# KdaiP/StableTTS

Hardware: AMD Instinct MI355X
Metric: mel-frames/sec (whole node), 31M DiT, n_timesteps=10+CFG (higher is better)
Workload: dtype f16

## Files before the change

stabletts_amd/csrc/attention.hip:

```cpp
#include "common.h"
#include "launch.h"

#if (defined(ST_ABL_NOEXP) || defined(ST_ABL_NOSUM)) && !defined(ST_DEVTOOLS)
#error "ST_ABL_* (ablation builds: results are garbage) need -DST_DEVTOOLS"
#endif
#ifdef ST_ABL_NOEXP
constexpr bool kAblNoExp = true;
#else
constexpr bool kAblNoExp = false;
#endif
#ifdef ST_ABL_NOSUM
constexpr bool kAblNoSum = true;
#else
constexpr bool kAblNoSum = false;
#endif
#ifndef ST_ATTN_WAVES
#define ST_ATTN_WAVES 8
#endif

namespace st {

template <class P, bool TRAIN, bool SPLIT = false, bool VLO = false>
__global__ __launch_bounds__(64 * ST_ATTN_WAVES, ST_ATTN_WAVES >= 16 || SPLIT ? 2 : 4) void attention_kernel(const AttnArgs a) {
    static_assert(!(TRAIN && SPLIT), "split-precision scores: inference kernel only");
    static_assert(!VLO || (TRAIN && !SPLIT), "hi + lo v: training kernel only");
    constexpr bool X3 = SPLIT || VLO;
    constexpr int NW = ST_ATTN_WAVES, QB = 32 * NW, QTILE = QB;
    using vec8 = typename P::vec8;
    constexpr int TILE_BYTES = 64 * 128;
    constexpr int NBUF = 3;
    constexpr int NT = X3 ? 3 : 2;
    constexpr int SMEM = NT * NBUF * TILE_BYTES > NW * 32 * 144 ? NT * NBUF * TILE_BYTES : NW * 32 * 144;
    __shared__ __attribute__((aligned(16))) unsigned char smem[SMEM];
    __shared__ float wave_lse[NW];
    unsigned char* Ks = smem;
    unsigned char* Vs = smem + NBUF * TILE_BYTES;
    unsigned char* KLs = smem + 2 * NBUF * TILE_BYTES;
    unsigned char* VLs = KLs;

    const int T = a.T, Tp = a.Tp, H = a.H;
    const int qtiles = (T + QB - 1) / QB;
    const int j = blockIdx.x >> 3;
    const int qt = j % qtiles, nh = (j / qtiles) * 8 + (blockIdx.x & 7);
    if (nh >= a.n_items * H) return;
    const int n = nh / H, h = nh % H;
    const int mb = n % a.mask_mod;
    if (a.t_lim && qt * QTILE >= a.t_lim[mb]) return;
    const int kvend = a.kv_end[mb];
    const int nfull = a.n_full[mb];
    const float* kbias = a.kbias + (size_t)mb * Tp;

    const int tid = threadIdx.x, lane = tid & 63;
    const int wave = __builtin_amdgcn_readfirstlane(tid >> 6);
    const int l31 = lane & 31, hi = lane >> 5;
    const int query = qt * QB + wave * 32 + l31;

    const unsigned char* qbase = (const unsigned char*)a.q + ((size_t)nh * T) * 128;
    const unsigned char* kbase = (const unsigned char*)a.k + ((size_t)nh * T) * 128;
    const unsigned char* vbase = (const unsigned char*)a.vt + ((size_t)nh * 64) * Tp * 2;
    const unsigned char* qlbase = SPLIT ? (const unsigned char*)a.q_lo + ((size_t)nh * T) * 128 : nullptr;
    const unsigned char* klbase = SPLIT ? (const unsigned char*)a.k_lo + ((size_t)nh * T) * 128 : nullptr;
    const unsigned char* vlbase = VLO ? (const unsigned char*)a.vt_lo + ((size_t)nh * 64) * Tp * 2 : nullptr;
    if constexpr (TRAIN) {
        if (qt * QB >= kvend) {
            if (query < T) {
                unsigned char* orow = (unsigned char*)a.out + (((size_t)n * T + query) * (H * 64) + h * 64) * 2 + hi * 64;
#pragma unroll
                for (int i = 0; i < 4; ++i) *(uint4*)(orow + 16 * i) = make_uint4(0, 0, 0, 0);
                if (hi == 0) a.lse[(size_t)nh * T + query] = 0.f;
            }
            return;
        }
    }

    vec8 qf[4];
#pragma unroll
    for (int ks = 0; ks < 4; ++ks) {
        uint4 v = make_uint4(0, 0, 0, 0);
        if (query < T) v = *(const uint4*)(qbase + (size_t)query * 128 + ks * 32 + hi * 16);
        qf[ks] = as_vec8<P>(v);
    }
    vec8 qlf[SPLIT ? 4 : 1];
    if constexpr (SPLIT) {
#pragma unroll
        for (int ks = 0; ks < 4; ++ks) {
            uint4 v = make_uint4(0, 0, 0, 0);
            if (query < T) v = *(const uint4*)(qlbase + (size_t)query * 128 + ks * 32 + hi * 16);
            qlf[ks] = as_vec8<P>(v);
        }
    }

    const int ntiles = (kvend + 63) >> 6;
    auto sgpr_ptr = [](const unsigned char* p) {
        const uintptr_t v = (uintptr_t)p;
        return (const unsigned char*)(((uintptr_t)(unsigned)__builtin_amdgcn_readfirstlane((int)(v >> 32)) << 32) |
                                      (unsigned)__builtin_amdgcn_readfirstlane((int)(unsigned)v));
    };
    auto issueKV = [&](int kt, int buf) {
        auto k_piece = [&](int piece) {
            int ln = lane;
            if constexpr (TRAIN) asm volatile("" : "+v"(ln));
            const int row = piece * 8 + (ln >> 3);
            const int seg = (ln & 7) ^ ((row >> 1) & 7);
            const int key = min(kt * 64 + row, T - 1);
            glds16s(sgpr_ptr(kbase), (unsigned)(key * 128 + seg * 16), Ks + buf * TILE_BYTES + piece * 1024);
            if constexpr (SPLIT) glds16s(sgpr_ptr(klbase), (unsigned)(key * 128 + seg * 16), KLs + buf * TILE_BYTES + piece * 1024);
        };
        auto v_piece = [&](int piece) {
            const int row = piece * 8 + (lane >> 3);
            const int seg = (lane & 7) ^ ((row >> 1) & 7);
            glds16s(sgpr_ptr(vbase + (size_t)kt * 128), (unsigned)((row * Tp + seg * 8) * 2), Vs + buf * TILE_BYTES + piece * 1024);
            if constexpr (VLO) glds16s(sgpr_ptr(vlbase + (size_t)kt * 128), (unsigned)((row * Tp + seg * 8) * 2), VLs + buf * TILE_BYTES + piece * 1024);
        };
        if constexpr (NW <= 8) {
#pragma unroll
            for (int k = 0; k < 8 / NW; ++k) { k_piece(wave * (8 / NW) + k); v_piece(wave * (8 / NW) + k); }
        } else {
            if (wave < 8) k_piece(wave); else v_piece(wave - 8);
        }
    };

    int row_off[2], swz[2];
#pragma unroll
    for (int b = 0; b < 2; ++b) {
        const int row = b * 32 + l31;
        row_off[b] = row * 128; swz[b] = (row >> 1) & 7;
    }

    f32x16_t o[2];
#pragma unroll
    for (int d = 0; d < 2; ++d)
#pragma unroll
        for (int r = 0; r < 16; ++r) o[d][r] = 0.f;
    constexpr float kBig = 8192.0f, kLazyTrain = 8.0f, kFloor = -20000.0f;
    unsigned drop_rh = 0;
    if constexpr (TRAIN) { if (a.drop.thresh16) drop_rh = a.drop.rowh[(size_t)nh * T + (query < T ? query : T - 1)]; }
    float m_ref = 0.f, l_run = 0.f;
    vec8 qaug, kaug;
#pragma unroll
    for (int i = 0; i < 8; ++i) { qaug[i] = to16<P>(0.f); kaug[i] = to16<P>(0.f); }
    if (hi == 0) kaug[0] = to16<P>(1.0f);

    if (ntiles > 0) issueKV(0, 0);
    if (ntiles > 1) { issueKV(1, 1); if constexpr (NW <= 8) { if constexpr (NW == 8) { if constexpr (X3) ST_DMA_WAIT(3); else ST_DMA_WAIT(2); } else { if constexpr (X3) ST_DMA_WAIT(6); else ST_DMA_WAIT(4); } } else ST_DMA_WAIT(1); }
    else ST_DMA_WAIT(0);
    __syncthreads();

    const int ntiles_run = ntiles;
    bool dead = false;
    if constexpr (!TRAIN) dead = a.t_lim && qt * QB + wave * 32 >= a.t_lim[mb];
    int buf = 0;
    for (int kt = 0; kt < ntiles_run; ++kt) {
        if (kt + 2 < ntiles_run) issueKV(kt + 2, buf >= 1 ? buf - 1 : NBUF - 1);
        if (!dead) {

        f32x16_t s[2];
        const bool partial = (kt + 1) * 64 > nfull;
        auto scores = [&]() __attribute__((always_inline)) {
#pragma unroll
            for (int kb = 0; kb < 2; ++kb) {
#pragma unroll
                for (int r = 0; r < 16; ++r) s[kb][r] = 0.f;
                s[kb] = P::mfma(kaug, qaug, s[kb]);
                const unsigned char* kp = Ks + buf * TILE_BYTES + row_off[kb];
#pragma unroll
                for (int ks = 0; ks < 4; ++ks) {
                    const vec8 kfrag = as_vec8<P>(*(const uint4*)(kp + (((ks * 2 + hi) ^ swz[kb]) << 4)));
                    s[kb] = P::mfma(kfrag, qf[ks], s[kb]);
                    if constexpr (SPLIT) {
                        s[kb] = P::mfma(kfrag, qlf[ks], s[kb]);
                        const unsigned char* klp = KLs + buf * TILE_BYTES + row_off[kb];
                        s[kb] = P::mfma(as_vec8<P>(*(const uint4*)(klp + (((ks * 2 + hi) ^ swz[kb]) << 4))), qf[ks], s[kb]);
                    }
                }
                __builtin_amdgcn_sched_barrier(0);
            }
            if (partial) {
#pragma unroll
                for (int kb = 0; kb < 2; ++kb)
#pragma unroll
                    for (int g4 = 0; g4 < 4; ++g4) {
                        const float4 bz = *(const float4*)(kbias + kt * 64 + kb * 32 + 8 * g4 + 4 * hi);
                        s[kb][4 * g4 + 0] += bz.x; s[kb][4 * g4 + 1] += bz.y;
                        s[kb][4 * g4 + 2] += bz.z; s[kb][4 * g4 + 3] += bz.w;
                    }
            }
        };
        vec8 pf[4];
        float psum[2];
        scores();
        if constexpr (TRAIN) {
            float mx = s[0][0];
#pragma unroll
            for (int kb = 0; kb < 2; ++kb)
#pragma unroll
                for (int r = 0; r < 16; ++r) mx = fmaxf(mx, s[kb][r]);
            mx = xor32_max(mx);
            if (kt == 0 || __any(mx > kLazyTrain)) {
                const bool need = kt == 0 || mx > kLazyTrain;
                const float m_new = need ? (float)to16<P>(fmaxf(m_ref + mx, kFloor)) : m_ref;
                const float alpha = kt == 0 ? 1.0f : __builtin_amdgcn_exp2f(m_ref - m_new);
                l_run *= alpha;
#pragma unroll
                for (int d = 0; d < 2; ++d)
#pragma unroll
                    for (int r = 0; r < 16; ++r) o[d][r] *= alpha;
                m_ref = m_new;
                if (hi == 0) qaug[0] = to16<P>(-m_ref);
                scores();
            }
            psum[0] = 0.f; psum[1] = 0.f;
#pragma unroll
            for (int kb = 0; kb < 2; ++kb)
#pragma unroll
                for (int g4 = 0; g4 < 4; ++g4) {
                    if (g4 == 2) __builtin_amdgcn_sched_barrier(0);
                    uint2 ch = make_uint2(0u, 0u);
                    if (a.drop.thresh16) ch = *(const uint2*)(a.drop.colh + ((kt * 64 + kb * 32 + 8 * g4 + 4 * hi) >> 1));
#pragma unroll
                    for (int h2 = 0; h2 < 2; ++h2) {
                        const int r = 4 * g4 + 2 * h2;
                        float p0 = __builtin_amdgcn_exp2f(s[kb][r]), p1 = __builtin_amdgcn_exp2f(s[kb][r + 1]);
                        psum[0] = add_f32_asm_safe(psum[0], p0);
                        psum[1] = add_f32_asm_safe(psum[1], p1);
                        if (a.drop.thresh16) {
                            const float2 f = drop_factors2(a.drop, drop_pair(drop_rh, h2 ? ch.y : ch.x));
                            p0 *= f.x; p1 *= f.y;
                        }
                        pf[kb * 2 + (r >> 3)][r & 7] = to16<P>(p0);
                        pf[kb * 2 + (r >> 3)][(r & 7) + 1] = to16<P>(p1);
                    }
                }
        } else {
            auto raise = [&](bool first) __attribute__((always_inline)) {
                float mx = s[0][0];
#pragma unroll
                for (int kb = 0; kb < 2; ++kb)
#pragma unroll
                    for (int r = 0; r < 16; ++r) mx = fmaxf(mx, s[kb][r]);
                mx = xor32_max(mx);
                const bool need = first || mx > 0.0f;
                const float m_new = need ? (float)to16<P>(fmaxf(m_ref + mx, kFloor)) : m_ref;
                const float alpha = first ? 1.0f : __builtin_amdgcn_exp2f(m_ref - m_new);
                l_run *= alpha;
#pragma unroll
                for (int d = 0; d < 2; ++d)
#pragma unroll
                    for (int r = 0; r < 16; ++r) o[d][r] *= alpha;
                m_ref = m_new;
                if (hi == 0) qaug[0] = to16<P>(-m_ref);
                scores();
            };
            auto numerators = [&]() __attribute__((always_inline)) {
                psum[0] = 0.f; psum[1] = 0.f;
#pragma unroll
                for (int kb = 0; kb < 2; ++kb)
#pragma unroll
                    for (int r = 0; r < 16; r += 2) {
                        float p0, p1;
                        if constexpr (kAblNoExp) { p0 = s[kb][r] * 0.001f; p1 = s[kb][r + 1] * 0.001f; }
                        else { p0 = __builtin_amdgcn_exp2f(s[kb][r]); p1 = __builtin_amdgcn_exp2f(s[kb][r + 1]); }
                        if constexpr (!kAblNoSum) {
                            psum[0] = add_f32_scalar(psum[0], p0);
                            psum[1] = add_f32_scalar(psum[1], p1);
                        }
                        pf[kb * 2 + (r >> 3)][r & 7] = to16<P>(p0);
                        pf[kb * 2 + (r >> 3)][(r & 7) + 1] = to16<P>(p1);
                    }
            };
            if (kt == 0) raise(true);
            numerators();
            if (kt != 0 && __any(!(psum[0] + psum[1] <= kBig))) {
                scores();
                raise(false);
                numerators();
            }
        }
        l_run += psum[0] + psum[1];

        __builtin_amdgcn_sched_barrier(0);
#pragma unroll
        for (int d = 0; d < 2; ++d) {
            const unsigned char* vp = Vs + buf * TILE_BYTES + row_off[d];
#pragma unroll
            for (int g = 0; g < 4; ++g)
                o[d] = P::mfma(as_vec8<P>(*(const uint4*)(vp + (((g * 2 + hi) ^ swz[d]) << 4))), pf[g], o[d]);
            if constexpr (VLO) {
                const unsigned char* vlp = VLs + buf * TILE_BYTES + row_off[d];
#pragma unroll
                for (int g = 0; g < 4; ++g)
                    o[d] = P::mfma(as_vec8<P>(*(const uint4*)(vlp + (((g * 2 + hi) ^ swz[d]) << 4))), pf[g], o[d]);
            }
        }
        }
        if (kt + 2 < ntiles_run) { if constexpr (NW <= 8) { if constexpr (NW == 8) { if constexpr (X3) ST_DMA_WAIT(3); else ST_DMA_WAIT(2); } else { if constexpr (X3) ST_DMA_WAIT(6); else ST_DMA_WAIT(4); } } else ST_DMA_WAIT(1); }
        else ST_DMA_WAIT(0);
        __syncthreads();
        buf = buf == NBUF - 1 ? 0 : buf + 1;
    }
    const float m_run = m_ref;
    const float l_tot = xor32_sum(l_run);
    const float inv = l_tot > 0.f ? 1.0f / l_tot : 0.f;
    if constexpr (!TRAIN) {
        if (a.lse_max) {
            float v = -3.0e38f;
            if (!dead && query < T && query < kvend && l_tot > 0.f) v = m_run + log2f(l_tot);
#pragma unroll
            for (int off = 16; off > 0; off >>= 1) v = fmaxf(v, __shfl_xor(v, off));
            if (lane == 0) wave_lse[wave] = v;
            __syncthreads();
            if (tid == 0) {
                float b = wave_lse[0];
#pragma unroll
                for (int w = 1; w < NW; ++w) b = fmaxf(b, wave_lse[w]);
                int bits = __float_as_int(b);
                bits = bits >= 0 ? bits : bits ^ 0x7fffffff;
                atomicMax((int*)a.lse_max + ((blockIdx.x % kLseCells) << 4), bits);
            }
        }
    }
    if (dead) return;
    if constexpr (TRAIN) {
        int lane_q = lane;
        asm volatile("" : "+v"(lane_q));
        const int query_e = qt * QB + wave * 32 + (lane_q & 31);
        if ((lane_q >> 5) == 0 && query_e < T) a.lse[(size_t)nh * T + query_e] = l_tot > 0.f ? m_run + log2f(l_tot) : 0.f;
    }
    unsigned char* mine = smem + wave * (32 * 144);
#pragma unroll
    for (int d = 0; d < 2; ++d)
#pragma unroll
        for (int q4 = 0; q4 < 4; ++q4)
            *(uint2*)(mine + l31 * 144 + (d * 32 + 8 * q4 + 4 * hi) * 2) =
                pack4<P>(o[d][4 * q4 + 0] * inv, o[d][4 * q4 + 1] * inv, o[d][4 * q4 + 2] * inv, o[d][4 * q4 + 3] * inv);
    const int rsub = lane >> 3, seg = lane & 7;
    unsigned char* obase = (unsigned char*)a.out + (((size_t)n * T + qt * QB + wave * 32) * (H * 64) + h * 64) * 2 + seg * 16;
#pragma unroll
    for (int i = 0; i < 4; ++i) {
        const int row = i * 8 + rsub;
        const uint4 v = *(const uint4*)(mine + row * 144 + seg * 16);
        if (qt * QB + wave * 32 + row < T) *(uint4*)(obase + (size_t)row * (H * 64) * 2) = v;
    }
}

constexpr int kAttnSmallLds = 8 * 2 * 64 * 128;
template <class P>
__global__ __launch_bounds__(512, 1) void attention_small_kernel(const AttnArgs a) {
    constexpr int NW = 8, TILE_BYTES = 64 * 128, WAVE_LDS = 2 * TILE_BYTES, OP = 33, QTILE = 32;
    using vec8 = typename P::vec8;
    extern __shared__ __attribute__((aligned(16))) unsigned char smem[];

    const int T = a.T, Tp = a.Tp, H = a.H;
    const int qgroups = (T + 31) / 32;
    const int total = a.n_items * H * qgroups;
    const int per_xcd = gridDim.x >> 3;
    const int lin = (blockIdx.x & 7) * per_xcd + (blockIdx.x >> 3);
    if (lin >= total) return;
    const int qt = lin % qgroups;
    const int nh = lin / qgroups;
    const int n = nh / H, h = nh % H;
    const int mb = n % a.mask_mod;
    if (a.t_lim && qt * QTILE >= a.t_lim[mb]) return;
    const int kvend = a.kv_end[mb];
    const int nfull = a.n_full[mb];
    const float* kbias = a.kbias + (size_t)mb * Tp;

    const int tid = threadIdx.x, lane = tid & 63;
    const int wave = __builtin_amdgcn_readfirstlane(tid >> 6);
    const int l31 = lane & 31, hi = lane >> 5;
    const int query = qt * 32 + l31;

    const unsigned char* qbase = (const unsigned char*)a.q + ((size_t)nh * T) * 128;
    const unsigned char* kbase = (const unsigned char*)a.k + ((size_t)nh * T) * 128;
    const unsigned char* vbase = (const unsigned char*)a.vt + ((size_t)nh * 64) * Tp * 2;
    const unsigned char* zeros = (const unsigned char*)a.zeros;
    unsigned char* Ks = smem + wave * WAVE_LDS;
    unsigned char* Vs = Ks + TILE_BYTES;
// ... 103 lines not shown
#pragma unroll
    for (int w = 0; w < NW; ++w) { mw[w] = ((const float*)(smem + w * WAVE_LDS))[64 * OP + q]; M = fmaxf(M, mw[w]); }
    float L = 0.f, acc[4] = {0.f, 0.f, 0.f, 0.f};
#pragma unroll
    for (int w = 0; w < NW; ++w) {
        const float* pw = (const float*)(smem + w * WAVE_LDS);
        const float sc = __builtin_amdgcn_exp2f(mw[w] - M);
        L += pw[64 * OP + 32 + q] * sc;
#pragma unroll
        for (int i = 0; i < 4; ++i) acc[i] += pw[(d0 + i) * OP + q] * sc;
    }
    const float inv = L > 0.f ? 1.0f / L : 0.f;
    if (qt * 32 + q < T)
        *(uint2*)((unsigned char*)a.out + (((size_t)n * T + qt * 32 + q) * (H * 64) + h * 64 + d0) * 2) =
            pack4<P>(acc[0] * inv, acc[1] * inv, acc[2] * inv, acc[3] * inv);
    if (a.lse_max) {
        __shared__ float wave_lse[NW];
        float v = -3.0e38f;
        if (qt * 32 + q < T && qt * 32 + q < kvend && L > 0.f) v = M + log2f(L);
#pragma unroll
        for (int off = 32; off > 0; off >>= 1) v = fmaxf(v, __shfl_xor(v, off));
        if (lane == 0) wave_lse[wave] = v;
        __syncthreads();
        if (tid == 0) {
            float b = wave_lse[0];
#pragma unroll
            for (int w = 1; w < NW; ++w) b = fmaxf(b, wave_lse[w]);
            int bits = __float_as_int(b);
            bits = bits >= 0 ? bits : bits ^ 0x7fffffff;
            atomicMax((int*)a.lse_max + ((blockIdx.x % kLseCells) << 4), bits);
        }
    }
}

template <class P>
static hipError_t launch_attention_small(const AttnArgs& a, hipStream_t s) {
    static bool attr_done_dev[64] = {};
    int dev_ = 0;
    if (hipGetDevice(&dev_) != hipSuccess || dev_ < 0 || dev_ >= 64) return hipErrorInvalidDevice;
    if (!attr_done_dev[dev_]) {
        hipError_t e = hipFuncSetAttribute((const void*)attention_small_kernel<P>, hipFuncAttributeMaxDynamicSharedMemorySize, kAttnSmallLds);
        if (e != hipSuccess) return e;
        attr_done_dev[dev_] = true;
    }
    const int total = a.n_items * a.H * ((a.T + 31) / 32);
    const int grid = ((total + 7) / 8) * 8;
    hipLaunchKernelGGL((attention_small_kernel<P>), dim3(grid), dim3(512), kAttnSmallLds, s, a);
    return hipGetLastError();
}

hipError_t launch_attention(int dtype, const AttnArgs& a, hipStream_t s) {
    if (!a.zeros || !a.kbias) return hipErrorInvalidValue;
    const int qtiles = (a.T + 32 * ST_ATTN_WAVES - 1) / (32 * ST_ATTN_WAVES);
    const int total = a.n_items * a.H * qtiles;
    if (!a.lse && !a.q_lo && a.small_max_blocks > 0 && total <= a.small_max_blocks)
        return dtype == DT_BF16 ? launch_attention_small<OpBF16>(a, s) : launch_attention_small<OpF16>(a, s);
    const int grid = 8 * ((a.n_items * a.H + 7) / 8) * qtiles;
    if (a.lse) {
        if (a.vt_lo) {
            if (dtype == DT_BF16) hipLaunchKernelGGL((attention_kernel<OpBF16, true, false, true>), dim3(grid), dim3(64 * ST_ATTN_WAVES), 0, s, a);
            else                  hipLaunchKernelGGL((attention_kernel<OpF16, true, false, true>), dim3(grid), dim3(64 * ST_ATTN_WAVES), 0, s, a);
            return hipGetLastError();
        }
        if (dtype == DT_BF16) hipLaunchKernelGGL((attention_kernel<OpBF16, true>), dim3(grid), dim3(64 * ST_ATTN_WAVES), 0, s, a);
        else                  hipLaunchKernelGGL((attention_kernel<OpF16, true>), dim3(grid), dim3(64 * ST_ATTN_WAVES), 0, s, a);
        return hipGetLastError();
    }
    if (a.q_lo || a.k_lo) {
        if (!a.q_lo || !a.k_lo) return hipErrorInvalidValue;
        static bool attr_done_dev[64][2] = {};
        int dev_ = 0;
        if (hipGetDevice(&dev_) != hipSuccess || dev_ < 0 || dev_ >= 64) return hipErrorInvalidDevice;
        const int di = dtype == DT_BF16 ? 0 : 1;
        const void* fn = di == 0 ? (const void*)attention_kernel<OpBF16, false, true> : (const void*)attention_kernel<OpF16, false, true>;
        if (!attr_done_dev[dev_][di]) {
            hipError_t e = hipFuncSetAttribute(fn, hipFuncAttributeMaxDynamicSharedMemorySize, 0);
            (void)e;
            attr_done_dev[dev_][di] = true;
        }
        if (di == 0) hipLaunchKernelGGL((attention_kernel<OpBF16, false, true>), dim3(grid), dim3(64 * ST_ATTN_WAVES), 0, s, a);
        else         hipLaunchKernelGGL((attention_kernel<OpF16, false, true>), dim3(grid), dim3(64 * ST_ATTN_WAVES), 0, s, a);
        return hipGetLastError();
    }
    if (dtype == DT_BF16) hipLaunchKernelGGL((attention_kernel<OpBF16, false>), dim3(grid), dim3(64 * ST_ATTN_WAVES), 0, s, a);
    else                  hipLaunchKernelGGL((attention_kernel<OpF16, false>), dim3(grid), dim3(64 * ST_ATTN_WAVES), 0, s, a);
    return hipGetLastError();
}

}
```

stabletts_amd/csrc/engine.cpp:

```cpp
#include "engine_dit.h"
#include "train_launch.h"
#include "mas_launch.h"
#include "align_train_launch.h"

#include <algorithm>
#include <cmath>
#include <cstdio>
#include <cstring>
#include <map>
#include <string>
#include <vector>

using namespace st;
using namespace sthost;

namespace sthost {
std::string g_create_error;

const char* kProfNames[PC_COUNT] = {
    "prep", "prenet_conv", "in_proj", "film_ln1", "qkv_rope", "attention", "out_proj", "ln2",
    "ffn_conv1", "ffn_conv2", "lsc_conv", "final_proj", "ode_update", "train_forward", "train_backward"};

int dev_alloc(st_engine* e, void** p, size_t bytes) {
    HIPCHK(e, hipMalloc(p, bytes ? bytes : 16));
// ... 341 lines not shown
    for (int i = 0; i < dit->L; ++i) {
        const std::string pre = "blocks." + std::to_string(i) + ".time_fusion.film.";
        HIPCHK(e, launch_linear(p.tau, p.n_t, C, P(e, pre + "weight"), P(e, pre + "bias"), 2 * C,
                                p.film + (size_t)i * p.n_t * 2 * C, 0, 0, s));
    }
    return ST_OK;
}

int run_estimator(st_engine* e, const Plan& p, const float* mask, int ev, hipStream_t s) {
    DitState* dit = dit_of(e);
    const int C = dit->C, F = dit->F, L = dit->L, N = p.N, T = p.T;
    const int64_t rowsC = (int64_t)N * T * C;
    const bool cap = e->capture;
    const bool dec = e->kind == KIND_DECODER;
    const bool film = dec;
    const bool skips = dec;
    const bool dec_fast_paths = dec;
    const bool split_qk = dec_fast_paths && dit->attn_split;
    const bool ragged = dec_fast_paths && e->tile.ragged_skip && !cap;
    const int ln1_by_ffn = skips ? L / 2 : L;
    auto ada_of = [&](int i) { return p.ada + (size_t)i * N * 6 * C; };
    auto fuse_ln1 = [&](ConvGemmArgs& a, int i) {
        a.ln_film = nullptr; a.ln_film_stride = 0; a.ln_film_mod = 1;
        if (film) {
            const float* fb = p.film + (size_t)i * p.n_t * 2 * C;
            if (ev >= 0) a.ln_film = fb + (size_t)ev * 2 * C;
            else         { a.ln_film = fb; a.ln_film_stride = 2 * C; a.ln_film_mod = p.B; }
        }
        a.ln_ada = ada_of(i); a.ln_ada_stride = 6 * C; a.ln_shift_off = 0; a.ln_scale_off = C;
        a.ln_mask_out = 0; a.ln_h16 = p.h16; a.mask = mask;
    };
    if (film) {
        ConvGemmArgs a = base_args(e, p, dit->inx, N);
        a.a0 = p.x16; a.c0 = dit->Mp; a.a0_mod = p.B; a.a1 = p.x16lo; a.c1 = dit->Mp; a.a1_mod = p.B; a.c2 = dit->Mp;
        a.bias = nullptr;
        a.add32 = p.cpart; a.add_clamp = p.B;
        a.out32 = p.X; a.out16 = p.skip16[0];
        fuse_ln1(a, 0);
        ProfScope ps(e, s, PC_INPROJ, conv_flops(p, dit->inx, N));
        HIPCHK(e, gemm(e, 1, EPI_F32, a, s));
    } else {
        FilmLnArgs a; memset(&a, 0, sizeof(a));
        a.X = p.X; a.h16 = p.h16; a.film = nullptr; a.film_mod = 1;
        a.ada = ada_of(0); a.ada_stride = 6 * C; a.shift_off = 0; a.scale_off = C;
        a.mask = mask; a.mask_mod = p.B; a.mask_out = 0; a.T = T; a.rows = N * T;
        ProfScope ps(e, s, PC_FILM_LN1, 0);
        HIPCHK(e, launch_film_ln(e->dt, a, s));
    }
    if (film && cap) capture(e, "h0", p.skip16[0], rowsC, true, s);
    for (int i = 0; i < L; ++i) {
        const std::string bn = "b" + std::to_string(i) + ".";
        const float* ada_i = ada_of(i);
        if (skips && i >= L / 2) {
            const int j = i - L / 2;
            ConvGemmArgs a = base_args(e, p, dit->lsc[j], N);
            a.a0 = p.cur16; a.c0 = C; a.a1 = p.skip16[L - 1 - i]; a.c1 = C;
            a.out32 = p.X;
            fuse_ln1(a, i);
            ProfScope ps(e, s, PC_LSC, conv_flops(p, dit->lsc[j], N));
            if (!(dit->skip_mask >> PC_LSC & 1)) HIPCHK(e, gemm(e, 3, EPI_F32, a, s));
        }
        if (cap) { capture(e, bn + "x1", p.X, rowsC, false, s); capture(e, bn + "h1", p.h16, rowsC, true, s); }
        {
            ConvGemmArgs a = base_args(e, p, dit->qkv[i], N);
            a.a0 = p.h16; a.c0 = C;
            a.q = p.q16; a.k = p.k16; a.vt = p.vt16; a.rope_cos = dit->rope_cos; a.rope_sin = dit->rope_sin;
            if (split_qk) { a.q_lo = p.q16lo; a.k_lo = p.k16lo; }
            a.Tp = p.Tp; a.n_heads = dit->H;
            if ((int)dit->qkv_frag.size() == L) a.w_frag = dit->qkv_frag[i];
            a.qscale = 1.4426950408889634f / sqrtf((float)(C / dit->H));
            ProfScope ps(e, s, PC_QKV, conv_flops(p, dit->qkv[i], N));
            if (!(dit->skip_mask >> PC_QKV & 1)) HIPCHK(e, gemm(e, 1, EPI_QKV, a, s));
        }
        if (cap) {
            capture(e, bn + "q", p.q16, rowsC, true, s); capture(e, bn + "k", p.k16, rowsC, true, s);
            capture(e, bn + "vt", p.vt16, (int64_t)N * C * p.Tp, true, s);
        }
        {
            AttnArgs a; memset(&a, 0, sizeof(a));
            a.q = p.q16; a.k = p.k16; a.vt = p.vt16; a.out = p.ao16; a.kbias = p.kbias; a.mask_mod = p.B; a.zeros = e->zeros;
            a.kv_end = p.kv_end; a.n_full = p.n_full; a.T = T; a.Tp = p.Tp; a.H = dit->H; a.n_items = N;
            a.small_max_blocks = dit->conc == 1 ? dit->attn_small_blocks : 0;
            if (split_qk) { a.q_lo = p.q16lo; a.k_lo = p.k16lo; }
            if (dec_fast_paths) a.lse_max = dit->lse_cells;
            if (ragged) a.t_lim = p.t_lim;
            ProfScope ps(e, s, PC_ATTN, 4.0 * (double)N * dit->H * (double)T * T * (C / dit->H));
            if (!(dit->skip_mask >> PC_ATTN & 1)) HIPCHK(e, launch_attention(e->dt, a, s));
        }
        if (cap) capture(e, bn + "attn", p.ao16, rowsC, true, s);
        const bool fused = dec_fast_paths && dit->fused_ffn && !cap && (int)dit->ffn_stream.size() == L && dit->ffn_stream[i] &&
                           (int64_t)dit->conc * N * ((T + kFfnFusedFrames - 1) / kFfnFusedFrames) >= e->tile.big_min_blocks;
        void* h2buf = fused ? p.h2_16 : p.h16;
        {
            ConvGemmArgs a = base_args(e, p, dit->oproj[i], N);
            a.a0 = p.ao16; a.c0 = C; a.mask = mask; a.gate = ada_i + 2 * C; a.gate_stride = 6 * C; a.out32 = p.X;
            a.ln_h16 = h2buf; a.ln_film = nullptr; a.ln_film_mod = 1;
            a.ln_ada = ada_i; a.ln_ada_stride = 6 * C; a.ln_shift_off = 3 * C; a.ln_scale_off = 4 * C; a.ln_mask_out = 1;
            if (dec_fast_paths && (int)dit->oproj_frag.size() == L && !cap) a.w_frag = dit->oproj_frag[i];
            ProfScope ps(e, s, PC_OPROJ, conv_flops(p, dit->oproj[i], N));
            if (!(dit->skip_mask >> PC_OPROJ & 1)) HIPCHK(e, gemm(e, 1, EPI_RESGATE, a, s));
        }
        if (cap) { capture(e, bn + "x2", p.X, rowsC, false, s); capture(e, bn + "h2", p.h16, rowsC, true, s); }
        if (!fused) {
            ConvGemmArgs a = base_args(e, p, dit->ffn1[i], N);
            a.a0 = p.h16; a.c0 = C; a.mask = mask; a.flags = GF_SILU | GF_MASK; a.out16 = p.u16;
            ProfScope ps(e, s, PC_FFN1, conv_flops(p, dit->ffn1[i], N));
            HIPCHK(e, gemm(e, 3, EPI_ACT16, a, s));
        }
        if (cap) capture(e, bn + "u", p.u16, (int64_t)N * T * F, true, s);
        void* copy16 = (skips && i + 1 < L / 2) ? p.skip16[i + 1] : p.cur16;
        {
            ConvGemmArgs a = base_args(e, p, dit->ffn2[i], N);
            a.a0 = p.u16; a.c0 = F; a.mask = mask; a.gate = ada_i + 5 * C; a.gate_stride = 6 * C; a.out32 = p.X;
            if (fused) { a.a0 = h2buf; a.c0 = C; a.w = dit->ffn_stream[i]; a.bias1 = dit->ffn1[i].bias; a.cmid = F; a.flags = GF_SILU | GF_MASK; }
            a.out16 = copy16;
            if (i + 1 == L) a.out16_lo = p.cur16lo;
            if (i + 1 < ln1_by_ffn) fuse_ln1(a, i + 1);
            else if (dec_fast_paths && !cap) a.out32_readonly = 1;
            ProfScope ps(e, s, PC_FFN2, conv_flops(p, dit->ffn2[i], N) + (fused ? conv_flops(p, dit->ffn1[i], N) : 0.0));
            if (dit->skip_mask >> PC_FFN2 & 1) {}
            else if (fused && dit->fused_ffn == 3) HIPCHK(e, launch_ffn_wino_f16(a, s));
            else if (fused) HIPCHK(e, e->dt == DT_BF16 ? launch_ffn_fused_bf16(a, s) : launch_ffn_fused_f16(a, s));
            else HIPCHK(e, gemm(e, 3, EPI_RESGATE, a, s));
        }
        if (cap) {
            if (film && i + 1 < ln1_by_ffn) capture(e, bn + "x3", copy16, rowsC, true, s);
            else capture(e, bn + "x3", p.X, rowsC, false, s);
        }
    }
    {
        ConvGemmArgs a = base_args(e, p, dit->fin, N);
        a.a0 = p.cur16; a.c0 = C; a.a1 = p.cur16lo; a.c1 = C; a.c2 = C; a.mask = mask; a.flags = GF_MASK; a.out32 = p.v32;
        ProfScope ps(e, s, PC_FINAL, conv_flops(p, dit->fin, N));
        HIPCHK(e, gemm(e, 1, EPI_F32, a, s));
    }
    if (cap) capture(e, "v", p.v32, (int64_t)N * T * dit->Mp, false, s);
    return ST_OK;
}

int check_handle(st_engine* e, Kind kind) {
    if (!e) return ST_ERR_INVALID;
    if (e->kind != kind)
        return e->fail(ST_ERR_STATE, std::string("this handle is not a ") + kKinds[kind].what + " (" + kKinds[kind].creator + ")");
    return ST_OK;
}

int check_finalized(st_engine* e) {
    return e->finalized ? ST_OK : e->fail(ST_ERR_STATE, "st_finalize() has not been called after loading parameters");
}

int check_sizes(st_engine* e, int B, int T, const char* t_name) {
    return B >= 1 && T >= 1 ? ST_OK : e->fail(ST_ERR_INVALID, std::string("B and ") + t_name + " must be >= 1");
}

int check_dropout(st_engine* e, float p_dropout) {
    return p_dropout >= 0.0f && p_dropout < 1.0f ? ST_OK : e->fail(ST_ERR_INVALID, "p_dropout must be in [0, 1)");
}

int check_ready(st_engine* e, Kind kind, int B, int T) {
    if (!e) return ST_ERR_INVALID;
    int rc = check_finalized(e); if (rc) return rc;
    if ((rc = check_sizes(e, B, T))) return rc;
    const DitState* dit = dit_or_null(e);
    if (dit && (int64_t)2 * B * T * dit->F >= (int64_t)1 << 31) return e->fail(ST_ERR_INVALID, "B*T too large for 32-bit row indexing");
    return check_handle(e, kind);
}
// ... 506 lines not shown
        return align_fail(ST_ERR_HIP, "align_train_backward kernel launch failed");
    return ST_OK;
}

int st_duration_loss_scratch_floats(void) { return kDurLossScratchFloats; }

int st_duration_loss(const float* logw, const int32_t* durations, const float* x_mask, const int64_t* x_lengths, int B, int Tx,
                     float* logw_target, float* scratch, float* loss, void* stream) {
    if (!logw || !durations || !x_mask || !x_lengths || !scratch || !loss) return align_fail(ST_ERR_INVALID, "null tensor pointer");
    if (B < 1 || Tx < 1) return align_fail(ST_ERR_INVALID, "shape out of range");
    if (launch_duration_loss(logw, durations, x_mask, (const long long*)x_lengths, B, Tx, logw_target, scratch, loss, (hipStream_t)stream) != hipSuccess)
        return align_fail(ST_ERR_HIP, "duration_loss kernel launch failed");
    return ST_OK;
}

int st_duration_loss_backward(const float* logw, const int32_t* durations, const float* x_mask, const float* scratch,
                              const float* grad_loss, int B, int Tx, float* grad_logw, void* stream) {
    if (!logw || !durations || !x_mask || !scratch || !grad_loss || !grad_logw) return align_fail(ST_ERR_INVALID, "null tensor pointer");
    if (B < 1 || Tx < 1) return align_fail(ST_ERR_INVALID, "shape out of range");
    if (launch_duration_loss_bwd(logw, durations, x_mask, scratch, grad_loss, B, Tx, grad_logw, (hipStream_t)stream) != hipSuccess)
        return align_fail(ST_ERR_HIP, "duration_loss_bwd kernel launch failed");
    return ST_OK;
}

int st_output_status(st_engine* e, void* stream, int* nonfinite) {
    if (!e) return ST_ERR_INVALID;
    if (!nonfinite) return e->fail(ST_ERR_INVALID, "null argument");
    DitState* dit = dit_or_null(e);
    if (!dit || !dit->status_host) return e->fail(ST_ERR_UNSUPPORTED, "host-mapped status word unavailable on this device");
    HIPCHK(e, hipSetDevice(e->device));
    HIPCHK(e, hipStreamSynchronize((hipStream_t)stream));
    *nonfinite = *dit->status_host != 0;
    dit->arena_poisoned(e);
    return ST_OK;
}

int st_cfm_loss_prep(const float* x1, const float* z, const float* t_rand, float sigma_min, int B, int M, int T, float* t, float* y,
                     float* u, void* stream) {
    if (!x1 || !z || !t_rand || !t || !y || !u) return align_fail(ST_ERR_INVALID, "null tensor pointer");
    if (B < 1 || M < 1 || T < 1 || B > 65535) return align_fail(ST_ERR_INVALID, "shape out of range");
    if (launch_cfm_loss_prep(x1, z, t_rand, sigma_min, B, M, T, t, y, u, (hipStream_t)stream) != hipSuccess)
        return align_fail(ST_ERR_HIP, "cfm_loss_prep kernel launch failed");
    return ST_OK;
}

int st_cfm_loss(const float* pred, const float* u, const float* mask, int B, int M, int T, float* scratch, float* loss, void* stream) {
    if (!pred || !u || !mask || !scratch || !loss) return align_fail(ST_ERR_INVALID, "null tensor pointer");
    if (B < 1 || M < 1 || T < 1) return align_fail(ST_ERR_INVALID, "shape out of range");
    if (launch_cfm_loss(pred, u, mask, B, M, T, scratch, loss, (hipStream_t)stream) != hipSuccess)
        return align_fail(ST_ERR_HIP, "cfm_loss kernel launch failed");
    return ST_OK;
}

int st_cfm_loss_backward(const float* pred, const float* u, const float* scratch, const float* grad_loss, int B, int M, int T,
                         float* grad_pred, void* stream) {
    if (!pred || !u || !scratch || !grad_loss || !grad_pred) return align_fail(ST_ERR_INVALID, "null tensor pointer");
    if (B < 1 || M < 1 || T < 1) return align_fail(ST_ERR_INVALID, "shape out of range");
    if (launch_cfm_loss_bwd(pred, u, scratch, grad_loss, B, M, T, grad_pred, (hipStream_t)stream) != hipSuccess)
        return align_fail(ST_ERR_HIP, "cfm_loss_bwd kernel launch failed");
    return ST_OK;
}

int st_cfm_loss_scratch_floats(void) { return 2 * kCfmLossBlocks + 2; }

int st_last_solve_stats(const st_engine* e, int64_t* nfe, int64_t* steps, int64_t* rejects) {
    if (!e) return ST_ERR_INVALID;
    const DitState* dit = dit_or_null(e);
    if (nfe) *nfe = dit ? dit->last_nfe : 0;
    if (steps) *steps = dit ? dit->last_steps : 0;
    if (rejects) *rejects = dit ? dit->last_rejects : 0;
    return ST_OK;
}

int st_set_option(st_engine* e, const char* name, int value) {
    if (!e || !name) return ST_ERR_INVALID;
    const std::string n(name);
    if (n == "attention_precision") {
        if (value != 0 && value != 1) return e->fail(ST_ERR_INVALID, "attention_precision: 0 (16-bit q / k operands) or 1 (split hi + lo operands)");
        if (e->kind != KIND_DECODER) return e->fail(ST_ERR_UNSUPPORTED, "attention_precision: CFM decoder handles only");
        DitState* dit = dit_of(e);
        if (value != dit->attn_split) { dit->drop_graphs(); dit->attn_split = value; }
        return ST_OK;
    }
    if (n == "fused_ffn") return e->fail(ST_ERR_INVALID, "fused_ffn is read-only (ST_FUSED_FFN at st_create)");
    return e->fail(ST_ERR_INVALID, std::string("unknown option: ") + name);
}

int st_get_option(const st_engine* e, const char* name, int* value) {
    if (!e || !name || !value) return ST_ERR_INVALID;
    const DitState* dit = dit_or_null(e);
    const std::string n(name);
    if (n == "attention_precision") { *value = dit ? dit->attn_split : 0; return ST_OK; }
    if (n == "fused_ffn") { *value = dit ? dit->fused_ffn : -1; return ST_OK; }
    return ST_ERR_INVALID;
}

int st_attention_stats(st_engine* e, void* stream, float* max_lse) {
    if (!e || !max_lse) return ST_ERR_INVALID;
    DitState* dit = dit_or_null(e);
    if (!dit || !dit->lse_cells) return e->fail(ST_ERR_STATE, "attention statistics unavailable (allocation failed at st_create)");
    HIPCHK(e, hipSetDevice(e->device));
    HIPCHK(e, hipStreamSynchronize((hipStream_t)stream));
    int cells[kLseCells * 16];
    HIPCHK(e, hipMemcpy(cells, dit->lse_cells, sizeof(cells), hipMemcpyDeviceToHost));
    int best = (int)0x80000000;
    for (int c = 0; c < kLseCells; ++c) best = std::max(best, cells[c * 16]);
    HIPCHK(e, hipMemsetD32((hipDeviceptr_t)dit->lse_cells, (int)0x80000000, kLseCells * 16));
    if (best == (int)0x80000000) { *max_lse = -INFINITY; return ST_OK; }
    const int bits = best >= 0 ? best : best ^ 0x7fffffff;
    float v; memcpy(&v, &bits, 4);
    *max_lse = v * 0.6931471805599453f;
    return ST_OK;
}

int st_debug_capture(st_engine* e, int enable) {
    if (!e) return ST_ERR_INVALID;
    e->capture = enable != 0;
    if (!enable) {
        hipSetDevice(e->device);
        hipDeviceSynchronize();
        for (auto& kv : e->caps) if (kv.second.dev) hipFree(kv.second.dev);
        e->caps.clear();
    }
    return ST_OK;
}

int64_t st_debug_fetch(st_engine* e, const char* name, float* host_out, int64_t capacity) {
    if (!e || !name) return ST_ERR_INVALID;
    auto it = e->caps.find(name);
    if (it == e->caps.end() || !it->second.dev) { e->err = std::string("no captured tensor named ") + name; return ST_ERR_INVALID; }
    Captured& c = it->second;
    if (!host_out) return c.n;
    if (capacity < c.n) { e->err = "capacity too small"; return ST_ERR_INVALID; }
    if (hipSetDevice(e->device) != hipSuccess || hipDeviceSynchronize() != hipSuccess) return ST_ERR_HIP;
    if (!c.is16) {
        if (hipMemcpy(host_out, c.dev, (size_t)c.n * 4, hipMemcpyDeviceToHost) != hipSuccess) return ST_ERR_HIP;
        return c.n;
    }
    float* tmp = nullptr;
    if (hipMalloc((void**)&tmp, (size_t)c.n * 4) != hipSuccess) return ST_ERR_HIP;
    hipError_t r = launch_cvt16_to_f32(e->dt, c.dev, tmp, c.n, nullptr);
    if (r == hipSuccess) r = hipMemcpy(host_out, tmp, (size_t)c.n * 4, hipMemcpyDeviceToHost);
    hipFree(tmp);
    return r == hipSuccess ? c.n : (int64_t)ST_ERR_HIP;
}

int st_profile_enable(st_engine* e, int enable) {
    if (!e) return ST_ERR_INVALID;
    hipSetDevice(e->device);
    prof_collect(e);
    e->prof = enable != 0;
    for (int i = 0; i < PC_COUNT; ++i) { e->prof_launches[i] = 0; e->prof_ms[i] = 0; e->prof_flops[i] = 0; }
    return ST_OK;
}

int st_profile_select(st_engine* e, uint64_t class_mask) {
    if (!e) return ST_ERR_INVALID;
    e->prof_mask = class_mask;
    return ST_OK;
}

int st_profile_stride(st_engine* e, int stride) {
    if (!e || stride < 1) return ST_ERR_INVALID;
    e->prof_stride = stride;
    for (int i = 0; i < PC_COUNT; ++i) e->prof_seen[i] = 0;
    return ST_OK;
}

int st_profile_num_classes(void) { return PC_COUNT; }

const char* st_profile_class_name(int cls) { return (cls >= 0 && cls < PC_COUNT) ? kProfNames[cls] : ""; }

int st_profile_read(st_engine* e, int cls, int64_t* launches, double* total_ms, double* flops_per_launch) {
    if (!e || cls < 0 || cls >= PC_COUNT) return ST_ERR_INVALID;
    hipSetDevice(e->device);
// ... 17 lines not shown
```

stabletts_amd/csrc/engine_dit.h:

```cpp
#pragma once
#include "engine_internal.h"
#include "stream_fork.h"

constexpr int kMaxParts = 1 + sthost::StreamFork::kMaxChildren;
constexpr size_t kSplitKBytes = 32u << 20;

namespace sthost {

struct TrainState;

struct DitState : KindState {
    st_config cfg{};
    bool dec = true;
    int M = 0, Mp = 0, C = 0, F = 0, H = 0, L = 0, K = 0, G = 0;
    int n_vocab = 0;
    std::string blk(int i) const { return dec ? "blocks." + std::to_string(i) + ".block." : "encoder." + std::to_string(i) + "."; }
    struct PackList { std::vector<st::PackJob> jobs; st::PackJob* dev = nullptr; unsigned nblocks = 0; bool ready = false; bool recording = false; };
    PackList pk_fwd, pk_T;
    bool packed_once = false;

    std::vector<Conv> pre;
    Conv inx, inc, fin;
    std::vector<Conv> lsc, qkv, oproj, ffn1, ffn2;
    std::vector<void*> oproj_frag;
    std::vector<void*> qkv_frag;
    std::vector<void*> ffn_stream;

    float* rope_cos = nullptr; float* rope_sin = nullptr; int rope_T = 0;
    void* sink = nullptr;

    int64_t last_nfe = 0, last_steps = 0, last_rejects = 0;
    int* status_host = nullptr; int* status_dev = nullptr;
    bool arena_poisoned(st_engine* e) { if (status_host && *status_host) { *status_host = 0; e->ws_sig = 0; return true; } return false; }

    void* adams_buf = nullptr; size_t adams_bytes = 0;
    unsigned skip_mask = 0;
    int qkv_ws_min_tiles = 400;
    int qkv_ws = 1;
    int oproj_ws = 1;
    int oproj_ws_min_tiles = 1000;
    int qkv_rc1 = 1;
    int fused_ffn = -1;
    int attn_split = 0;
    unsigned* lse_cells = nullptr;
    int attn_small_blocks = 32;
    int conc = 1;
    StreamFork part_streams;

    struct SolveGraph {
        int B, T, n_steps, solver, use_cfg; float cfg_strength; const char* ws; int parts; int seen; hipGraphExec_t exec;
    };
    std::vector<SolveGraph> graphs;
    hipStream_t gstream = nullptr;
    void drop_graphs() {
        for (auto& g : graphs) if (g.exec) hipGraphExecDestroy(g.exec);
        graphs.clear();
    }

    TrainState* train = nullptr;

    ~DitState() override;
    int finalize(st_engine* e) override;
    int repack(st_engine* e, hipStream_t s) override;
    int64_t device_bytes() const override;
    int64_t train_serial() const override;
    void params_moved() override { pk_fwd.ready = false; pk_T.ready = false; drop_graphs(); }
    void arena_moved() override { drop_graphs(); }
};

inline DitState* dit_of(st_engine* e) { return state_of<DitState>(e); }
inline const DitState* dit_of(const st_engine* e) { return state_of<DitState>(e); }
inline const DitState* dit_or_null(const st_engine* e) { return e->kind == KIND_DECODER || e->kind == KIND_TEXT_ENCODER ? dit_of(e) : nullptr; }
inline DitState* dit_or_null(st_engine* e) { return const_cast<DitState*>(dit_or_null(const_cast<const st_engine*>(e))); }

int arena_fresh(st_engine* e, uint64_t sig, size_t used_bytes, hipStream_t s);
int ensure_rope(st_engine* e, int T, hipStream_t s);
int check_ready(st_engine* e, Kind kind, int B, int T);
int pack_all(st_engine* e, hipStream_t s);
bool pk_replay(st_engine* e, DitState::PackList& L, hipStream_t s, int* rc);
void pk_begin(DitState::PackList& L);
int pk_end(st_engine* e, DitState::PackList& L, hipStream_t s);
int pk_weight(st_engine* e, DitState::PackList& L, const float* src, int cout, int cin_total, int K, int ci_off, int ci_cnt, void* dst,
              int row_off, int cin_p, int col_off, int slice_w, int lo, hipStream_t s);
int pk_weight_t(st_engine* e, DitState::PackList& L, const float* src, int cout, int cin_total, int taps, int ci_off, int ci_cnt, void* dst,
                int cin_p, int ld, int col_off, hipStream_t s);
int pk_copy(st_engine* e, DitState::PackList& L, float* dst, const float* src, int n, hipStream_t s);

struct Plan {
    int B, T, Tp, N, Pn, n_t;
    bool cfg;
    void *mu16, *pre1, *pre2, *cond16, *cond16lo, *x16, *x16lo, *h16, *h2_16, *q16, *k16, *q16lo, *k16lo, *vt16, *ao16, *u16, *cur16, *cur16lo;
    void* skip16[8];
    float *cpart, *X, *v32, *xstate, *kbuf[7], *ynew, *ode_partial, *ode_out, *tvals, *emb, *th, *tau, *film, *cvec, *ada, *ada_tmp;
    int *n_full, *kv_end;
    int* t_lim;
    float* kbias;
    float* maskbuf;
    struct Slot { void** dst; size_t off; };
    std::vector<Slot> slots;
};
size_t layout_plan(st_engine* e, int B, int T, bool cfg, int n_t, size_t off, Plan* p);
void bind_plan(st_engine* e, Plan* p);
uint64_t layout_sig(int entry, int B, int T, int cfg, int n_t, int parts);
int run_prenet(st_engine* e, const Plan& p, hipStream_t s);
int run_adaln(st_engine* e, const Plan& p, hipStream_t s);
int run_time_tables(st_engine* e, const Plan& p, hipStream_t s);
int run_estimator(st_engine* e, const Plan& p, const float* mask, int ev, hipStream_t s);

int train_prepare(st_engine* e, hipStream_t s);
void train_invalidate(DitState* dit);
void train_destroy(DitState* dit);
int64_t train_bytes(const DitState* dit);

}
```

stabletts_amd/csrc/launch.h:

```cpp
#pragma once
#include <hip/hip_runtime.h>
#include <stdint.h>

namespace st {

enum { DT_BF16 = 0, DT_F16 = 1 };

enum { EPI_ACT16 = 0, EPI_F32 = 1, EPI_RESGATE = 2, EPI_QKV = 3,
       EPI_GELU16 = 4,
       EPI_SILU = 5 };
enum { GF_SILU = 1, GF_MASK = 2,
       GF_K2_V_ONLY = 4 };

struct ConvGemmArgs {
    const void* a0; const void* a1;
    int c0, c1;
    int c2;
    int a0_mod, a1_mod;
    const void* w;
    long long w_item_stride;
    const float* bias;
    int cout, T, n_items;
    int tiles_f, tiles_c;
    const float* mask; int mask_mod;
    int flags;
    void* out16; float* out32;
    int out32_readonly;
    void* out16_lo;
    const float* add32; int add_clamp;
    const float* gate; int gate_stride;
    const float* res32;
    float* branch32;
    void* q; void* k; void* vt;
    void* q_lo; void* k_lo;
    void* vt_lo;
    const float* rope_cos; const float* rope_sin;
    int Tp; float qscale; int n_heads;
    const void* zeros;
    const void* w_frag;
    void* sink;
    void* ln_h16;
    const float* ln_film; int ln_film_stride; int ln_film_mod;
    const float* ln_ada; int ln_ada_stride; int ln_shift_off; int ln_scale_off;
    int ln_mask_out;
    const int* t_lim; int t_lim_mod;
    void* act16; const void* dact16;
    unsigned long long drop_seed; unsigned drop_thresh16; float drop_scale;
    int ksplit;
    const float* bias1; int cmid;
    unsigned long long* dbg;
};

enum { G2_T128 = 0, G2_RC = 1, G2_K3PIPE = 2,
       G2_BIG = 3,
       G2_T64 = 4, G2_RC64 = 5,
       G2_PHASED = 6,
       G2_RC1 = 7 };
hipError_t launch_conv_gemm2_bf16(int cfg, int taps, int epi, const ConvGemmArgs& a, hipStream_t s);
hipError_t launch_conv_gemm2_f16(int cfg, int taps, int epi, const ConvGemmArgs& a, hipStream_t s);
hipError_t launch_splitk_finish_bf16(int epi, const ConvGemmArgs& a, const float* part, int S, hipStream_t s);
hipError_t launch_splitk_finish_f16(int epi, const ConvGemmArgs& a, const float* part, int S, hipStream_t s);
constexpr int kFfnFusedFrames = 126;
hipError_t launch_ffn_fused_bf16(const ConvGemmArgs& a, hipStream_t s);
hipError_t launch_ffn_fused_f16(const ConvGemmArgs& a, hipStream_t s);
hipError_t launch_pack_ffn_stream(int dtype, const float* src, int stage, int F, void* dst, hipStream_t s);
hipError_t launch_pack_ffn_wino(const float* src, int stage, int F, void* dst, hipStream_t s);
hipError_t launch_ffn_wino_f16(const ConvGemmArgs& a, hipStream_t s);
hipError_t launch_qkv_ws(int dtype, const ConvGemmArgs& a, hipStream_t s);
hipError_t launch_oproj_ws(int dtype, const ConvGemmArgs& a, hipStream_t s);
hipError_t launch_pack_qkv_frag(int dtype, const float* src, int plane, void* dst, hipStream_t s);
constexpr int kGemmFramesPerTile = 128;
constexpr int kGemmChannelsPerTile = 128;

struct DropCfg { unsigned long long seed; unsigned thresh16; float scale; const unsigned* rowh; const unsigned* colh; };

struct AttnArgs {
    const void* q; const void* k; const void* vt; void* out;
    const void* q_lo; const void* k_lo;
    const void* vt_lo;
    unsigned* lse_max;
    const float* kbias; int mask_mod;
    const int* kv_end; const int* n_full;
    int T, Tp, H, n_items;
    const void* zeros;
    float* lse;
    DropCfg drop;
    const int* t_lim;
    int small_max_blocks;
};
constexpr int kLseCells = 16;
hipError_t launch_attention(int dtype, const AttnArgs& a, hipStream_t s);

struct FilmLnArgs {
    float* X;
    void* h16;
    const float* film; int film_stride; int film_mod;
    const float* ada; int ada_stride;
    int shift_off, scale_off;
    const float* mask; int mask_mod;
    int mask_out;
    int T, rows;
};
hipError_t launch_film_ln(int dtype, const FilmLnArgs& a, hipStream_t s);

hipError_t launch_time_embed(const float* t, int n_t, int dim, float* emb, hipStream_t s);
hipError_t launch_silu_rows(const float* in, int64_t n, float* out, hipStream_t s);
struct LinearJobs { const float* in[8]; const float* W[8]; const float* bias[8]; float* out[8]; int n; };
hipError_t launch_linear_multi(const LinearJobs& J, int n, int k, int o, int silu_in, int silu_out, hipStream_t s);
hipError_t launch_linear(const float* in, int n, int k, const float* W, const float* bias, int o,
                         float* out, int silu_in, int silu_out, hipStream_t s);
constexpr int kFrameHalo = 4;
hipError_t launch_mask_prep(const float* mask, int B, int T, int Tp, int* n_full, int* kv_end, float* kbias, int* t_lim, hipStream_t s);

hipError_t launch_to_time_major(int dtype, const float* in, int B, int C, int T, int Cp,
                                float* out32, void* out16, void* out16lo, hipStream_t s);
hipError_t launch_from_time_major(const float* in, int B, int C, int T, int Cp, float* out, hipStream_t s, int* nonfinite = nullptr);
hipError_t launch_embed_tokens(const long long* tokens, const long long* lengths, const float* emb, int n_vocab,
                               int C, float scale, int B, int T, float* X, float* mask_out, hipStream_t s);
hipError_t launch_set_values(float* dst, const float* host_vals, int n, hipStream_t s);
hipError_t launch_delay(int us, hipStream_t s);
hipError_t launch_cvec_prep(const float* c, const float* fake_or_null, int B, int G, float* dst, hipStream_t s);
hipError_t launch_fill_rows16(int dtype, const float* vec, int C, int Cp, int T, void* out16, hipStream_t s);

hipError_t launch_cfg_combine(int dtype, const float* v, int B, int64_t per_item, int use_cfg, float s,
                              float* kout, float* xio, void* x16, void* x16lo, float dt, hipStream_t stream);
hipError_t launch_lincomb(int dtype, const float* x, const float* const* k, const float* coef, int nk,
                          int64_t n, float* y32, void* y16, void* y16lo, hipStream_t s);

hipError_t launch_pack_weight(int dtype, const float* src, int cout, int cin_total, int K, int ci_off,
                              int ci_cnt, void* dst, int row_off, int cin_p, int col_off, int slice_w, int lo,
                              hipStream_t s);
hipError_t launch_cvt16_to_f32(int dtype, const void* src, float* dst, int64_t n, hipStream_t s);
struct PackJob { const float* src; void* dst; int kind, cout, cin_total, K, ci_off, ci_cnt, row_off, cin_p, col_off, slice_w, lo; unsigned blk0; };
hipError_t launch_pack_jobs(int dtype, const PackJob* jobs_dev, int njobs, unsigned nblocks, hipStream_t s);

constexpr int kCfmLossBlocks = 1024;
hipError_t launch_cfm_loss_prep(const float* x1, const float* z, const float* t_rand, float sigma_min, int B, int M, int T,
                                float* t_out, float* y, float* u, hipStream_t s);
hipError_t launch_cfm_loss(const float* pred, const float* u, const float* mask, int B, int M, int T, float* scratch, float* loss, hipStream_t s);
hipError_t launch_cfm_loss_bwd(const float* pred, const float* u, const float* scratch, const float* grad_loss, int B, int M, int T, float* gpred, hipStream_t s);

hipError_t launch_durations(const float* logw, const float* x_mask, float length_scale, int B, int Tx, float* w_ceil,
                            float* cum, long long* y_len, hipStream_t s);
hipError_t launch_cumsum_rows(const float* dur, int B, int Tx, float* cum, hipStream_t s);
hipError_t launch_path(const float* cum, const float* mask, int B, int Tx, int Ty, float* path, hipStream_t s);
hipError_t launch_align(const float* cum, const float* x_mask, const long long* y_len, const float* mu_x, int B, int M, int Tx,
                        int Ty, float* attn, float* mu_y, float* y_mask, hipStream_t s);

hipError_t launch_set_scalar(float* dst, float v, hipStream_t s);
struct OdeNormArgs { const float* y; const float* a; const float* b; const float* k[7]; float coef[7]; int nk;
                     float rtol, atol; int64_t n; int mode; float* partial; float* out; };
hipError_t launch_ode_norm(const OdeNormArgs& a, hipStream_t s);
constexpr int kOdeNormBlocks = 1024;
hipError_t launch_dopri5_interp(const float* y0, const float* y1, const float* const* k, const float* cmid_dt, float dt,
                                float x, int64_t n, float* out, hipStream_t s);

}
```

Measured before the change: 1.321 million.

## Stage attention K/V in 128-key pairs with four LDS buffers and fewer barriers

Adds a KSTAGE=128 variant of the inference attention kernel. It uses four 64-key LDS buffers in dynamic shared memory, prefetches two tiles at a time and waits for DMA and synchronizes only every other tile, halving the block barriers. It also restructures the QK score loop to preload K fragments and interleave loads with MFMAs. The variant is the default for the decoder. The cost is more LDS per block, which may lower occupancy, and a longer wait when each pair of tiles is issued.

```diff
diff --git a/stabletts_amd/csrc/attention.hip b/stabletts_amd/csrc/attention.hip
--- a/stabletts_amd/csrc/attention.hip
+++ b/stabletts_amd/csrc/attention.hip
@@ -20,18 +20,23 @@
 
 namespace st {
 
-template <class P, bool TRAIN, bool SPLIT = false, bool VLO = false>
+template <class P, bool TRAIN, bool SPLIT = false, bool VLO = false, int KSTAGE = 64>
 __global__ __launch_bounds__(64 * ST_ATTN_WAVES, ST_ATTN_WAVES >= 16 || SPLIT ? 2 : 4) void attention_kernel(const AttnArgs a) {
     static_assert(!(TRAIN && SPLIT), "split-precision scores: inference kernel only");
     static_assert(!VLO || (TRAIN && !SPLIT), "hi + lo v: training kernel only");
+    static_assert(KSTAGE == 64 || (KSTAGE == 128 && !TRAIN && !SPLIT && !VLO && ST_ATTN_WAVES <= 8), "128-key stages: the 16-bit inference kernel only");
+    constexpr bool K2 = KSTAGE == 128;
     constexpr bool X3 = SPLIT || VLO;
     constexpr int NW = ST_ATTN_WAVES, QB = 32 * NW, QTILE = QB;
     using vec8 = typename P::vec8;
     constexpr int TILE_BYTES = 64 * 128;
-    constexpr int NBUF = 3;
+    constexpr int NBUF = K2 ? 4 : 3;
     constexpr int NT = X3 ? 3 : 2;
     constexpr int SMEM = NT * NBUF * TILE_BYTES > NW * 32 * 144 ? NT * NBUF * TILE_BYTES : NW * 32 * 144;
-    __shared__ __attribute__((aligned(16))) unsigned char smem[SMEM];
+    static_assert(!K2 || SMEM == kAttnKstage128Lds, "launch_attention sets this many bytes of dynamic LDS");
+    __shared__ __attribute__((aligned(16))) unsigned char smem_static[K2 ? 16 : SMEM];
+    extern __shared__ __attribute__((aligned(16))) unsigned char attn_dyn_smem[];
+    unsigned char* smem = K2 ? attn_dyn_smem : smem_static;
     __shared__ float wave_lse[NW];
     unsigned char* Ks = smem;
     unsigned char* Vs = smem + NBUF * TILE_BYTES;
@@ -142,21 +147,48 @@
     if (hi == 0) kaug[0] = to16<P>(1.0f);
 
     if (ntiles > 0) issueKV(0, 0);
-    if (ntiles > 1) { issueKV(1, 1); if constexpr (NW <= 8) { if constexpr (NW == 8) { if constexpr (X3) ST_DMA_WAIT(3); else ST_DMA_WAIT(2); } else { if constexpr (X3) ST_DMA_WAIT(6); else ST_DMA_WAIT(4); } } else ST_DMA_WAIT(1); }
+    if constexpr (K2) { if (ntiles > 1) issueKV(1, 1); ST_DMA_WAIT(0); }
+    else if (ntiles > 1) { issueKV(1, 1); if constexpr (NW <= 8) { if constexpr (NW == 8) { if constexpr (X3) ST_DMA_WAIT(3); else ST_DMA_WAIT(2); } else { if constexpr (X3) ST_DMA_WAIT(6); else ST_DMA_WAIT(4); } } else ST_DMA_WAIT(1); }
     else ST_DMA_WAIT(0);
     __syncthreads();
+    if constexpr (!TRAIN && !SPLIT) asm volatile("" :: "v"(qf[0]), "v"(qf[1]), "v"(qf[2]), "v"(qf[3]));
 
     const int ntiles_run = ntiles;
     bool dead = false;
     if constexpr (!TRAIN) dead = a.t_lim && qt * QB + wave * 32 >= a.t_lim[mb];
     int buf = 0;
     for (int kt = 0; kt < ntiles_run; ++kt) {
+        if constexpr (K2) {
+            if (!(kt & 1)) {
+                const int nsub = min(2, ntiles_run - (kt + 2));
+#pragma nounroll
+                for (int u = 0; u < nsub; ++u) issueKV(kt + 2 + u, (buf ^ 2) + u);
+            }
+        } else
         if (kt + 2 < ntiles_run) issueKV(kt + 2, buf >= 1 ? buf - 1 : NBUF - 1);
         if (!dead) {
 
         f32x16_t s[2];
         const bool partial = (kt + 1) * 64 > nfull;
         auto scores = [&]() __attribute__((always_inline)) {
+            if constexpr (!TRAIN && !SPLIT) {
+                const unsigned char* kp = Ks + buf * TILE_BYTES;
+                auto kread = [&](int i) { return as_vec8<P>(*(const uint4*)(kp + row_off[i >> 2] + ((((i & 3) * 2 + hi) ^ swz[i >> 2]) << 4))); };
+                vec8 kf[8];
+#pragma unroll
+                for (int i = 0; i < 4; ++i) kf[i] = kread(i);
+#pragma unroll
+                for (int r = 0; r < 16; ++r) { s[0][r] = 0.f; s[1][r] = 0.f; }
+                s[0] = P::mfma(kaug, qaug, s[0]);
+                s[1] = P::mfma(kaug, qaug, s[1]);
+                __builtin_amdgcn_sched_barrier(0);
+#pragma unroll
+                for (int i = 0; i < 8; ++i) {
+                    s[i >> 2] = P::mfma(kf[i], qf[i & 3], s[i >> 2]);
+                    if (i + 4 < 8) kf[i + 4] = kread(i + 4);
+                    __builtin_amdgcn_sched_barrier(0);
+                }
+            } else {
 #pragma unroll
             for (int kb = 0; kb < 2; ++kb) {
 #pragma unroll
@@ -174,6 +206,7 @@
                     }
                 }
                 __builtin_amdgcn_sched_barrier(0);
+            }
             }
             if (partial) {
 #pragma unroll
@@ -293,6 +326,11 @@
             }
         }
         }
+        if constexpr (K2) {
+            if ((kt & 1) || kt + 1 == ntiles_run) { ST_DMA_WAIT(0); __syncthreads(); }
+            buf = (buf + 1) & 3;
+            continue;
+        }
         if (kt + 2 < ntiles_run) { if constexpr (NW <= 8) { if constexpr (NW == 8) { if constexpr (X3) ST_DMA_WAIT(3); else ST_DMA_WAIT(2); } else { if constexpr (X3) ST_DMA_WAIT(6); else ST_DMA_WAIT(4); } } else ST_DMA_WAIT(1); }
         else ST_DMA_WAIT(0);
         __syncthreads();
@@ -562,6 +600,22 @@
         else         hipLaunchKernelGGL((attention_kernel<OpF16, false, true>), dim3(grid), dim3(64 * ST_ATTN_WAVES), 0, s, a);
         return hipGetLastError();
     }
+    if (a.kstage == 128) {
+        static bool attr_done_dev[64][2] = {};
+        int dev_ = 0;
+        if (hipGetDevice(&dev_) != hipSuccess || dev_ < 0 || dev_ >= 64) return hipErrorInvalidDevice;
+        const int di = dtype == DT_BF16 ? 0 : 1;
+        const void* fn = di == 0 ? (const void*)attention_kernel<OpBF16, false, false, false, 128> : (const void*)attention_kernel<OpF16, false, false, false, 128>;
+        if (!attr_done_dev[dev_][di]) {
+            hipError_t e = hipFuncSetAttribute(fn, hipFuncAttributeMaxDynamicSharedMemorySize, kAttnKstage128Lds);
+            if (e != hipSuccess) return e;
+            attr_done_dev[dev_][di] = true;
+        }
+        if (di == 0) hipLaunchKernelGGL((attention_kernel<OpBF16, false, false, false, 128>), dim3(grid), dim3(64 * ST_ATTN_WAVES), kAttnKstage128Lds, s, a);
+        else         hipLaunchKernelGGL((attention_kernel<OpF16, false, false, false, 128>), dim3(grid), dim3(64 * ST_ATTN_WAVES), kAttnKstage128Lds, s, a);
+        return hipGetLastError();
+    }
+    if (a.kstage != 0 && a.kstage != 64) return hipErrorInvalidValue;
     if (dtype == DT_BF16) hipLaunchKernelGGL((attention_kernel<OpBF16, false>), dim3(grid), dim3(64 * ST_ATTN_WAVES), 0, s, a);
     else                  hipLaunchKernelGGL((attention_kernel<OpF16, false>), dim3(grid), dim3(64 * ST_ATTN_WAVES), 0, s, a);
     return hipGetLastError();
diff --git a/stabletts_amd/csrc/engine.cpp b/stabletts_amd/csrc/engine.cpp
--- a/stabletts_amd/csrc/engine.cpp
+++ b/stabletts_amd/csrc/engine.cpp
@@ -447,6 +447,7 @@
             a.kv_end = p.kv_end; a.n_full = p.n_full; a.T = T; a.Tp = p.Tp; a.H = dit->H; a.n_items = N;
             a.small_max_blocks = dit->conc == 1 ? dit->attn_small_blocks : 0;
             if (split_qk) { a.q_lo = p.q16lo; a.k_lo = p.k16lo; }
+            a.kstage = dit->attn_kstage;
             if (dec_fast_paths) a.lse_max = dit->lse_cells;
             if (ragged) a.t_lim = p.t_lim;
             ProfScope ps(e, s, PC_ATTN, 4.0 * (double)N * dit->H * (double)T * T * (C / dit->H));
@@ -1119,6 +1120,13 @@
         if (value != dit->attn_split) { dit->drop_graphs(); dit->attn_split = value; }
         return ST_OK;
     }
+    if (n == "attn_kstage") {
+        if (value != 64 && value != 128) return e->fail(ST_ERR_INVALID, "attn_kstage: 64 or 128 keys per stage");
+        if (e->kind != KIND_DECODER) return e->fail(ST_ERR_UNSUPPORTED, "attn_kstage: CFM decoder handles only");
+        DitState* dit = dit_of(e);
+        if (value != dit->attn_kstage) { dit->drop_graphs(); dit->attn_kstage = value; }
+        return ST_OK;
+    }
     if (n == "fused_ffn") return e->fail(ST_ERR_INVALID, "fused_ffn is read-only (ST_FUSED_FFN at st_create)");
     return e->fail(ST_ERR_INVALID, std::string("unknown option: ") + name);
 }
@@ -1128,6 +1136,7 @@
     const DitState* dit = dit_or_null(e);
     const std::string n(name);
     if (n == "attention_precision") { *value = dit ? dit->attn_split : 0; return ST_OK; }
+    if (n == "attn_kstage") { *value = dit ? dit->attn_kstage : 128; return ST_OK; }
     if (n == "fused_ffn") { *value = dit ? dit->fused_ffn : -1; return ST_OK; }
     return ST_ERR_INVALID;
 }
diff --git a/stabletts_amd/csrc/engine_dit.h b/stabletts_amd/csrc/engine_dit.h
--- a/stabletts_amd/csrc/engine_dit.h
+++ b/stabletts_amd/csrc/engine_dit.h
@@ -42,6 +42,7 @@
     int qkv_rc1 = 1;
     int fused_ffn = -1;
     int attn_split = 0;
+    int attn_kstage = 128;
     unsigned* lse_cells = nullptr;
     int attn_small_blocks = 32;
     int conc = 1;
diff --git a/stabletts_amd/csrc/launch.h b/stabletts_amd/csrc/launch.h
--- a/stabletts_amd/csrc/launch.h
+++ b/stabletts_amd/csrc/launch.h
@@ -87,8 +87,10 @@
     DropCfg drop;
     const int* t_lim;
     int small_max_blocks;
+    int kstage;
 };
 constexpr int kLseCells = 16;
+constexpr int kAttnKstage128Lds = 2 * 4 * 64 * 128;
 hipError_t launch_attention(int dtype, const AttnArgs& a, hipStream_t s);
 
 struct FilmLnArgs {
```

After: 1.325 million (median of 6 runs). Within noise of the previous version (+0.3%).
